# facebookresearch/ReAgent

Hardware: NVIDIA H100
Metric: minibatch_td_updates_per_sec_b4096 (higher is better)
Workload: dtype f32

## Files before the change

profiles/time_k2.py:

```python
import argparse
import json
import os
import statistics
import sys
import tempfile

ROOT = os.path.dirname(os.path.dirname(os.path.abspath(__file__)))
if ROOT not in sys.path:
    sys.path.insert(0, ROOT)

from profiles.timing import (alternate, capture, card_info, cuda_device,
                             replay_us, write_result)

CTAS = (1, 8, 32, 64, 128)
ARRANGEMENTS = {"k1_on_side_stream": True, "one_stream": False}


def k2_graph(trainer, rb, rows, A, launches):
    from reagent_b200 import _lib

    batch = rb.sample_discrete_dqn_batch(rows, A)
    trainer.train_batch(batch)
    qd, qtd, a, wsc, keep, pack = trainer._last_td_call
    assert pack is not None, "config-2 shapes run K2 on the wgmma path"
    alive = (trainer._ws, keep, batch, pack)
    lib = _lib.lib()

    def launch():
        _lib.check(lib.rb200_dqn_td_step_tc(qd, qtd, a, wsc, pack.data_ptr(), pack.numel(), 1,
                                            _lib.cur_stream()), "rb200_dqn_td_step_tc")

    return capture(launch, launches), alive


def draw(rb, n, B, dev):
    import numpy as np
    import torch

    out = np.empty((n, B), dtype=np.float64)
    for i in range(n):
        qv, pos, _ = rb.host_queries(B)
        while pos:
            qv, pos, _ = rb.host_queries(B)
        out[i] = qv
    return torch.from_numpy(out).to(dev)


def kernel_class(name):
    if "dqn_td_tc" in name:
        return "K2"
    if "wgrad" in name:
        return "wgrad"
    if "adam" in name:
        return "adam"
    if "sample" in name or "draw" in name:
        return "K1"
    return "other"


def breakdown(g, steps, tmp, tag):
    import torch
    from torch.profiler import ProfilerActivity, profile

    g.replay()
    torch.cuda.synchronize()
    with profile(activities=[ProfilerActivity.CUDA]) as prof:
        g.replay()
        torch.cuda.synchronize()
    path = os.path.join(tmp, f"k2_{tag}.pt.trace.json")
    prof.export_chrome_trace(path)
    with open(path) as f:
        ev = [e for e in json.load(f)["traceEvents"]
              if e.get("cat") == "kernel" and e.get("ph") == "X"]
    ev.sort(key=lambda e: e["ts"])
    dur, gap, last_end = {}, {}, {}
    for e in ev:
        c = kernel_class(e["name"])
        s = e.get("args", {}).get("stream", -1)
        dur.setdefault(c, []).append(e["dur"])
        if s in last_end:
            gap.setdefault(c, []).append(e["ts"] - last_end[s])
        last_end[s] = e["ts"] + e["dur"]
    k2 = [e["ts"] for e in ev if kernel_class(e["name"]) == "K2"]
    period = [b - a for a, b in zip(k2, k2[1:])]
    return {
        "kernels_per_update": {c: len(v) / steps for c, v in dur.items()},
        "names": sorted({e["name"][:120] for e in ev}),
        "median_us": {c: statistics.median(v) for c, v in dur.items()},
        "median_gap_before_on_same_stream_us": {c: statistics.median(v) for c, v in gap.items()},
        "median_k2_start_to_start_us": statistics.median(period) if period else None,
    }


def main():
    ap = argparse.ArgumentParser()
    ap.add_argument("--out", required=True, help="directory for the result file")
    ap.add_argument("--reps", type=int, default=11)
    ap.add_argument("--launches", type=int, default=200)
    ap.add_argument("--steps", type=int, default=100)
    args = ap.parse_args()

    dev = cuda_device(__file__)
    import torch

    import bench
    from reagent_b200.replay_memory import PrioritizedReplayBuffer
    from reagent_b200.training.fused_step import capture_device_only

    cfg = dict(bench.CONFIGS[2])
    B, A = cfg["B"], cfg["A"]
    info = card_info()
    rb = PrioritizedReplayBuffer(stack_size=1, replay_capacity=cfg["cap"], batch_size=B, device=dev)
    rb.add_batch(**bench.synth_stream(cfg["cap"], 1000, cfg))
    trainer = bench.build_trainer(cfg, dev)

    graphs, alive = {}, []
    for n in CTAS:
        graphs[n], keep = k2_graph(trainer, rb, 32 * n, A, args.launches)
        alive.append(keep)
    k2 = alternate(CTAS, args.reps, lambda n, rep: replay_us(graphs[n], args.launches))
    del graphs
    sweep = {str(n): {s: v[s] for s in ("median", "min", "max")} for n, v in k2.items()}

    for _ in range(3):
        trainer.train_batch(rb.sample_discrete_dqn_batch(B, A))
    torch.cuda.synchronize()
    steps = {k: capture_device_only(trainer, rb, B, args.steps, draw(rb, args.steps, B, dev),
                                    overlap_sampling=ov) for k, ov in ARRANGEMENTS.items()}
    per_update = alternate(steps, args.reps, lambda k, rep: replay_us(steps[k], args.steps))
    with tempfile.TemporaryDirectory() as tmp:
        traced = {k: breakdown(g, args.steps, tmp, k) for k, g in steps.items()}

    one, full = sweep["1"]["median"], sweep[str(CTAS[-1])]["median"]
    res = {
        "what": ("dqn_td_tc_kernel (K2) at config-2 shapes: alone at 32 rows per CTA over a "
                 "sweep of CTA counts; the captured config-2 step kernel by kernel and per "
                 "update, with the sample kernel (K1) of the next update on a second stream "
                 "(bench.py's graph) and with all kernels on one stream"),
        "card": info,
        "config": dict(B=B, S=cfg["S"], A=A, sizes=cfg["sizes"], double_q=True, loss="huber"),
        "method": (f"K2: CUDA events around one replay of a graph of {args.launches} launches "
                   f"(weights prepacked), captured after 5 warm-up launches on a side stream, "
                   f"{args.reps} alternating repetitions, medians; step: CUDA events around one "
                   f"replay of a {args.steps}-update capture_device_only graph, {args.reps} "
                   f"alternating repetitions; every timed replay after an untimed one; "
                   f"breakdown: torch.profiler (CUDA activities) over one replay of the same "
                   f"graphs, in a separate pass"),
        "k2_alone_us_by_ctas": sweep,
        "k2_128_over_1_cta": full / one,
        "step_per_update_us": per_update,
        "step_breakdown": traced,
    }
    write_result(args.out, __file__, res)


if __name__ == "__main__":
    main()
```

reagent_b200/csrc/rb200_dqn_tc.cu:

```cuda
#include <string.h>

#include "rb200_dqn_tc_layout.cuh"
#include "rb200_wgmma.cuh"

namespace rb200 {

constexpr int kQR = 32;
constexpr int kQSub = 2;
constexpr int kQStages = 3;
constexpr int kQStageBytes = kQSub * (kQKC / 4) * kQFullLbo;
constexpr int kQLboB = 64 * 16 + 16;
constexpr int kQLoOff = 32 * 4;
constexpr int kQEpiThreads = 256;
constexpr int kQThreads = kQEpiThreads + 32;
constexpr int kQMaxTiles = 4;
constexpr int kQMaxSteps = 4 * kMaxLayers;
constexpr int kQMaxSmem = 232448;
static_assert(kQKC == 32, "a chunk is four K = 8 MMA steps");

enum { kStepHidden = 0, kStepLast = 1, kStepBwd = 2 };

struct QStep {
  uint32_t pack_off;
  int16_t N, K;
  int8_t layer, kind, net, in_buf, load_x, save, qdst, out_buf;
};

struct QDev {
  rb200_dqn_args_t a;
  rb200_net_ws_t ws;
  const unsigned char* pack;
  int nsteps, last_fwd_step;
  int buf_off[3];
  int q_off, ldq, lin_off, bar_off;
  int need_zero;
  QStep steps[kQMaxSteps];
};

struct PackJob {
  const float* W;
  int N, K;
  int ld;
  int transpose;
  uint32_t pack_off;
  int chunk0;
};
struct PackDev {
  PackJob jobs[3 * kMaxLayers];
  int njobs;
  unsigned char* pack;
};

constexpr int kPackParts = 4;

__global__ void __launch_bounds__(256) dqn_tc_pack_kernel(const PackDev p) {
  const int chunk = (int)blockIdx.x / kPackParts, part = (int)blockIdx.x % kPackParts;
  int j = 0;
  while (j + 1 < p.njobs && chunk >= p.jobs[j + 1].chunk0) ++j;
  const PackJob job = p.jobs[j];
  const int local = chunk - job.chunk0;
  const int kch = ceil_div(job.K, kQKC);
  const int t = local / kch, c = local - t * kch;
  const ChunkGeo g = chunk_geo(job.N, job.K, t, c);
  const int rows8 = (int)(g.lbo - 16) / 16, kl8 = g.ksteps * 8;
  float* img = reinterpret_cast<float*>(p.pack + job.pack_off + g.off);
  const int m0 = 128 * t, k0 = kQKC * c;
  const int total = rows8 * kl8;
  constexpr int U = 4;
  for (int base = (part * 256 + (int)threadIdx.x); base < total; base += kPackParts * 256 * U) {
    float v[U];
    int o[U];
#pragma unroll
    for (int u = 0; u < U; ++u) {
      const int idx = base + u * kPackParts * 256;
      int m, kk;
      if (job.transpose) { kk = idx / rows8; m = idx - kk * rows8; }
      else { m = idx / kl8; kk = idx - m * kl8; }
      v[u] = 0.f;
      o[u] = -1;
      if (idx < total) {
        o[u] = (kk >> 2) * (int)(g.lbo / 4) + m * 4 + (kk & 3);
        if (m0 + m < job.N && k0 + kk < job.K)
          v[u] = job.transpose ? __ldg(job.W + (size_t)(k0 + kk) * job.ld + m0 + m)
                               : __ldg(job.W + (size_t)(m0 + m) * job.ld + k0 + kk);
      }
    }
#pragma unroll
    for (int u = 0; u < U; ++u)
      if (o[u] >= 0) img[o[u]] = v[u];
  }
}

__device__ __noinline__ float act_fwd_slow(float x, int act) { return act_fwd(x, act); }
__device__ __noinline__ float act_bwd_slow(float y, int act) { return act_bwd_from_out(y, act); }

template <bool kWeighted>
__global__ void __launch_bounds__(kQThreads, 1)
dqn_td_tc_kernel(const Mlp q, const Mlp qt, const QDev p) {
  extern __shared__ __align__(128) unsigned char smem_raw[];
  const int tid = threadIdx.x, warp = tid >> 5, lane = tid & 31;
  const rb200_dqn_args_t& a = p.a;
  const int B = a.batch;
  const int row0 = blockIdx.x * kQR;
  const int L = q.n_layers;
  const int A = q.dims[L];

  if (p.need_zero) {
    unsigned nbytes;
    asm("mov.u32 %0, %%dynamic_smem_size;" : "=r"(nbytes));
    for (unsigned i = (unsigned)p.buf_off[0] + tid * 16u; i + 15u < nbytes; i += kQThreads * 16u)
      *reinterpret_cast<float4*>(smem_raw + i) = make_float4(0.f, 0.f, 0.f, 0.f);
  }
  __syncthreads();

  unsigned char* ring = smem_raw;
  float* qarr = reinterpret_cast<float*>(smem_raw + p.q_off);
  float* act_s = reinterpret_cast<float*>(smem_raw + p.lin_off);
  float* mask_s = act_s + kQR * A;
  float* scal_s = mask_s + kQR * A;
  uint64_t* full = reinterpret_cast<uint64_t*>(smem_raw + p.bar_off);
  uint64_t* sfree = full + kQStages;
  const int ldq = p.ldq;

  if (tid == 0) {
    for (int s = 0; s < kQStages; ++s) { mbar_init(full + s, 1); mbar_init(sfree + s, kQEpiThreads / 32); }
    asm volatile("fence.mbarrier_init.release.cluster;\n" ::: "memory");
  }
  __syncthreads();

  const int role = __shfl_sync(0xffffffffu, warp, 0);
  if (role == kQEpiThreads / 32) {
    const bool leader = elect_one();
    int stage = 0;
    uint32_t par = 1;
    for (int s = 0; s < p.nsteps; ++s) {
      const QStep st = p.steps[s];
      const int mt = ceil_div(st.N, 128), kch = ceil_div(st.K, kQKC);
      const uint32_t tile_stride = (uint32_t)(round_up8(st.K) / 4) * kQFullLbo;
      for (int t = 0; t < mt; ++t) {
        const int rows = st.N - 128 * t;
        const uint32_t lbo = (uint32_t)(round_up8(rows < 128 ? rows : 128) * 16 + 16);
        const uint32_t full_bytes = (kQKC / 4) * lbo;
        const int klast = st.K - kQKC * (kch - 1);
        const uint32_t last_bytes = (uint32_t)(round_up8(klast) / 4) * lbo;
        const unsigned char* src = p.pack + st.pack_off + (size_t)t * tile_stride;
        for (int c = 0; c < kch; c += kQSub) {
          const int nsub = kch - c < kQSub ? kch - c : kQSub;
          const uint32_t bytes = (uint32_t)(nsub - 1) * full_bytes + ((c + nsub == kch) ? last_bytes : full_bytes);
          mbar_wait(sfree + stage, par);
          if (leader) {
            mbar_expect_tx(full + stage, bytes);
            bulk_g2s(ring + stage * kQStageBytes, src, bytes, full + stage);
          }
          src += bytes;
          if (++stage == kQStages) { stage = 0; par ^= 1u; }
        }
      }
    }
  } else {
    const int wg = warp >> 2, w4 = warp & 3, g = lane >> 2, tq = lane & 3;
    int ss = 0;
    uint32_t spar = 0;

    constexpr int kXQ = 4;
    const int xS = q.dims[0];
    const int xnq = round_up8(xS) / 4;
    const bool x_in_regs = kQR * xnq <= kXQ * kQEpiThreads;
    float4 xr[kXQ];
    auto x_fetch_one = [&](const float* src, int idx) {
      const bool vec = ((xS & 3) == 0) && ((reinterpret_cast<uintptr_t>(src) & 15) == 0);
      const int r = idx / xnq, qd = idx - r * xnq;
      const int k = 4 * qd, row = row0 + r;
      float4 v = make_float4(0.f, 0.f, 0.f, 0.f);
      if (idx < kQR * xnq && row < B) {
        const float* sp = src + (size_t)row * xS;
        if (vec && k + 3 < xS) {
          asm volatile("ld.global.nc.v4.f32 {%0,%1,%2,%3}, [%4];\n"
                       : "=f"(v.x), "=f"(v.y), "=f"(v.z), "=f"(v.w)
                       : "l"(sp + k));
        } else {
          if (k < xS) v.x = sp[k];
          if (k + 1 < xS) v.y = sp[k + 1];
          if (k + 2 < xS) v.z = sp[k + 2];
          if (k + 3 < xS) v.w = sp[k + 3];
        }
      }
      return v;
    };
    auto x_store_one = [&](int idx, const float4 v) {
      if (idx >= kQR * xnq) return;
      float* base = reinterpret_cast<float*>(smem_raw + p.buf_off[0]);
      const int r = idx / xnq, qd = idx - r * xnq;
      float4 h, l;
      split4(v, h, l);
      const int o = qd * (kQLboB / 4) + r * 4;
      *reinterpret_cast<float4*>(base + o) = h;
      *reinterpret_cast<float4*>(base + o + kQLoOff) = l;
    };
    auto x_fetch = [&](const float* src) {
      if (!x_in_regs) return;
#pragma unroll
      for (int i = 0; i < kXQ; ++i) xr[i] = x_fetch_one(src, tid + i * kQEpiThreads);
    };
    auto x_store = [&](const float* src) {
      if (x_in_regs) {
#pragma unroll
        for (int i = 0; i < kXQ; ++i) x_store_one(tid + i * kQEpiThreads, xr[i]);
      } else {
        for (int idx = tid; idx < kQR * xnq; idx += kQEpiThreads) x_store_one(idx, x_fetch_one(src, idx));
      }
    };
    auto load_loss_inputs = [&]() {
      const float* mask = a.maxq ? a.possible_next_actions_mask : a.next_action;
      for (int idx = tid; idx < kQR * A; idx += kQEpiThreads) {
        const int r = idx / A;
        const bool in = row0 + r < B;
        const size_t g = (size_t)row0 * A + idx;
        act_s[idx] = in ? a.action[g] : 0.f;
        mask_s[idx] = (in && mask) ? mask[g] : 1.f;
      }
      if (tid < kQR) {
        const int row = row0 + tid;
        const bool in = row < B;
        scal_s[tid * 4 + 0] = in ? a.reward[row] : 0.f;
        scal_s[tid * 4 + 1] = in ? a.not_terminal[row] : 0.f;
        scal_s[tid * 4 + 2] = (in && a.discount_mode == RB200_DISCOUNT_POW) ? a.discount_src[row] : 0.f;
      }
    };
    auto step_tiles = [&](const QStep& st) {
      const Mlp& net = st.net ? qt : q;
      const int l = st.layer, N = st.N;
      const int mt = ceil_div(N, 128), kch = ceil_div(st.K, kQKC);
      float* obase = reinterpret_cast<float*>(smem_raw + p.buf_off[st.out_buf]);
      const uint32_t bbase = smem_u32(smem_raw + p.buf_off[st.in_buf]);
      for (int t = 0; t < mt; ++t) {
        const int rows = N - 128 * t;
        const int rows8 = round_up8(rows < 128 ? rows : 128);
        const uint32_t lbo = (uint32_t)(rows8 * 16 + 16);
        const bool live = 64 * wg < rows;
        const int m0 = 64 * wg + 16 * w4 + g;
        const bool ok0 = live && m0 < rows8, ok1 = live && m0 + 8 < rows8;
        float acc[32];
#pragma unroll
        for (int i = 0; i < 32; ++i) acc[i] = 0.f;
        for (int c = 0; c < kch; c += kQSub) {
          const int nsub = kch - c < kQSub ? kch - c : kQSub;
          mbar_wait(full + ss, spar);
          uint32_t ah[kQSub * 4][4], al[kQSub * 4][4];
          int ksteps[kQSub];
#pragma unroll
          for (int j = 0; j < kQSub; ++j) {
            const int kl = st.K - kQKC * (c + j);
            ksteps[j] = j < nsub ? round_up8(kl < kQKC ? kl : kQKC) / 8 : 0;
            const unsigned char* src = ring + ss * kQStageBytes + (uint32_t)j * (kQKC / 4) * lbo + tq * 4;
#pragma unroll
            for (int ks = 0; ks < 4; ++ks) {
              float v[4] = {0.f, 0.f, 0.f, 0.f};
              if (ks < ksteps[j]) {
                const unsigned char* s0 = src + (uint32_t)(2 * ks) * lbo;
                const unsigned char* s1 = s0 + lbo;
                if (ok0) { v[0] = *reinterpret_cast<const float*>(s0 + m0 * 16); v[2] = *reinterpret_cast<const float*>(s1 + m0 * 16); }
                if (ok1) { v[1] = *reinterpret_cast<const float*>(s0 + (m0 + 8) * 16); v[3] = *reinterpret_cast<const float*>(s1 + (m0 + 8) * 16); }
              }
#pragma unroll
              for (int e = 0; e < 4; ++e) {
                float h, lo_;
                split1(v[e], h, lo_);
                ah[4 * j + ks][e] = __float_as_uint(h);
                al[4 * j + ks][e] = __float_as_uint(lo_);
              }
            }
          }
          __syncwarp();
          if (lane == 0) mbar_arrive(sfree + ss);
          if (++ss == kQStages) { ss = 0; spar ^= 1u; }
          wgmma_fence();
#pragma unroll
          for (int j = 0; j < kQSub; ++j) {
#pragma unroll
            for (int ks = 0; ks < 4; ++ks) {
              if (ks < ksteps[j]) {
                const uint32_t kq = (uint32_t)(2 * (4 * (c + j) + ks));
                const uint64_t bd = wgmma_desc(bbase + kq * kQLboB, kQLboB, 128);
                wgmma_rs_n64(acc, ah[4 * j + ks], bd, 1u);
                wgmma_rs_n32(acc, al[4 * j + ks], bd, 1u);
              }
            }
          }
          wgmma_commit();
          wgmma_wait<0>();
        }
        if (!live) continue;

#pragma unroll
        for (int hh = 0; hh < 2; ++hh) {
          const int n = 128 * t + m0 + 8 * hh;
          const bool valid = n < N;
          float x[8];
#pragma unroll
          for (int i = 0; i < 4; ++i)
#pragma unroll
            for (int e = 0; e < 2; ++e) x[2 * i + e] = acc[4 * i + 2 * hh + e] + acc[4 * (i + 4) + 2 * hh + e];
          auto rowof = [&](int k) { return 8 * (k >> 1) + 2 * tq + (k & 1); };
          float* ob = obase + (n >> 2) * (kQLboB / 4) + (n & 3);
          bool to_operand, to_global;
          float* gdst = nullptr;
          if (st.kind == kStepBwd) {
            const int hact = q.act[l - 1];
            float hv[8];
            if (st.save) {
              const float* hs = p.ws.hidden[l - 1];
#pragma unroll
              for (int k = 0; k < 8; ++k) {
                const int row = row0 + rowof(k);
                hv[k] = (valid && row < B) ? hs[(size_t)row * N + n] : 0.f;
              }
            } else {
#pragma unroll
              for (int k = 0; k < 8; ++k) hv[k] = valid ? ob[rowof(k) * 4] + ob[rowof(k) * 4 + kQLoOff] : 0.f;
            }
            if (hact == RB200_ACT_RELU) {
#pragma unroll
              for (int k = 0; k < 8; ++k) x[k] = hv[k] > 0.f ? x[k] : 0.f;
            } else if (hact != RB200_ACT_LINEAR) {
#pragma unroll
              for (int k = 0; k < 8; ++k) x[k] = valid ? x[k] * act_bwd_slow(hv[k], hact) : 0.f;
            }
            to_operand = l - 1 >= 1;
            to_global = true;
            gdst = p.ws.dz[l - 1];
          } else {
            const float bias = valid ? __ldg(net.params + net.b_off[l] + n) : 0.f;
            const int act = net.act[l];
            if (act == RB200_ACT_RELU) {
#pragma unroll
              for (int k = 0; k < 8; ++k) x[k] = fmaxf(x[k] + bias, 0.f);
            } else if (act == RB200_ACT_LINEAR) {
#pragma unroll
              for (int k = 0; k < 8; ++k) x[k] += bias;
            } else {
#pragma unroll
              for (int k = 0; k < 8; ++k) x[k] = act_fwd_slow(x[k] + bias, act);
            }
            to_operand = st.kind != kStepLast;
            to_global = st.save != 0 && st.kind != kStepLast;
            gdst = to_global ? p.ws.hidden[l] : nullptr;
          }
          if (!valid) continue;
          if (st.kind == kStepLast) {
            float* qd = qarr + st.qdst * kQR * ldq + n;
#pragma unroll
            for (int k = 0; k < 8; ++k) qd[rowof(k) * ldq] = x[k];
            continue;
          }
          if (to_operand) {
#pragma unroll
            for (int k = 0; k < 8; ++k) {
              float h, lo_;
              split1(row0 + rowof(k) < B ? x[k] : 0.f, h, lo_);
              ob[rowof(k) * 4] = h;
              ob[rowof(k) * 4 + kQLoOff] = lo_;
            }
          }
          if (to_global) {
#pragma unroll
            for (int k = 0; k < 8; ++k) {
              const int row = row0 + rowof(k);
              if (row < B) gdst[(size_t)row * N + n] = x[k];
            }
          }
        }
      }
    };
    auto loss_stage = [&]() {
      const float* qa = qarr;
      const float* qb = qarr + kQR * ldq;
      const float* qc = qarr + 2 * kQR * ldq;
      const int r = tid >> 3, sub = tid & 7;
      const int row = row0 + r;
      const bool in = row < B;
      float best = 0.f, sel = 0.f, qsel = 0.f, bsum = 0.f;
      int bi = 0x7fffffff;
      for (int c = sub; c < A; c += 8) {
        const float pen = -1e9f * (1.f - mask_s[r * A + c]);
        const float vt = qb[r * ldq + c] + pen;
        const float key = a.double_q ? (qa[r * ldq + c] + pen) : vt;
        if (bi == 0x7fffffff || key > best) { best = key; bi = c; sel = vt; }
        const float aw = act_s[r * A + c];
        qsel += qc[r * ldq + c] * aw;
        if (a.reward_boost) bsum += aw * a.reward_boost[c];
      }
#pragma unroll
      for (int o = 1; o < 8; o <<= 1) {
        const float ob = __shfl_xor_sync(0xffffffffu, best, o);
        const float os = __shfl_xor_sync(0xffffffffu, sel, o);
        const int oi = __shfl_xor_sync(0xffffffffu, bi, o);
        qsel += __shfl_xor_sync(0xffffffffu, qsel, o);
        bsum += __shfl_xor_sync(0xffffffffu, bsum, o);
        if (oi != 0x7fffffff && (bi == 0x7fffffff || ob > best || (ob == best && oi < bi))) {
          best = ob; bi = oi; sel = os;
        }
      }
      float le = 0.f, g = 0.f;
      if (in) {
        const float rew = scal_s[r * 4 + 0] + bsum;
        const float disc = (a.discount_mode == RB200_DISCOUNT_POW)
                               ? powf(a.gamma, scal_s[r * 4 + 2]) : a.gamma;
        const float tgt = rew + disc * (sel * scal_s[r * 4 + 1]);
        const float d = qsel - tgt;
        const float invB = 1.f / (float)B;
        if (a.loss_kind == RB200_LOSS_HUBER) {
          const float ad = fabsf(d);
          le = ad < 1.f ? 0.5f * d * d : ad - 0.5f;
          g = (d < -1.f) ? -invB : (d > 1.f ? invB : invB * d);
        } else {
          le = d * d;
          g = 2.f * invB * d;
        }
        if (kWeighted) {
          const float w = a.sample_weight[row];
          le *= w;
          g *= w;
        }
        if (sub == 0) {
          if (a.td_target) a.td_target[row] = tgt;
          if (a.next_action_idx) a.next_action_idx[row] = bi;
          if (a.q_selected) a.q_selected[row] = qsel;
        }
      }
      const int A8 = round_up8(A);
      const int lact = q.act[L - 1];
      float* zb = reinterpret_cast<float*>(smem_raw + p.buf_off[2]) + r * 4;
      for (int c = sub; c < A8; c += 8) {
        float v = 0.f;
        if (in && c < A) {
          v = g * act_s[r * A + c];
          if (lact != RB200_ACT_LINEAR) v *= act_bwd_slow(qc[r * ldq + c], lact);
          if (a.all_action_scores) a.all_action_scores[(size_t)row * A + c] = qc[r * ldq + c];
          if (a.do_backward) p.ws.dz[L - 1][(size_t)row * A + c] = v;
        }
        if (a.do_backward) {
          float h, lo_;
          split1(v, h, lo_);
          float* o = zb + (c >> 2) * (kQLboB / 4) + (c & 3);
          o[0] = h;
          o[kQLoOff] = lo_;
        }
      }
      const float ws = warp_sum(sub == 0 ? le : 0.f);
      if (lane == 0) scal_s[kQR * 4 + warp] = ws;
    };


    auto x_src = [&](int lx) { return lx == 1 ? a.state : a.next_state; };
    auto handover = [&]() {
      fence_proxy_async_smem();
      asm volatile("bar.sync 1, %0;\n" ::"n"(kQEpiThreads) : "memory");
    };
    if (p.steps[0].load_x) { x_fetch(x_src(p.steps[0].load_x)); x_store(x_src(p.steps[0].load_x)); }
    load_loss_inputs();
    handover();
    for (int s = 0; s < p.nsteps; ++s) {
      const QStep st = p.steps[s];
      const int lx = (s + 1 < p.nsteps) ? p.steps[s + 1].load_x : 0;
      if (lx) x_fetch(x_src(lx));
      step_tiles(st);
      handover();
      if (s == p.last_fwd_step) {
        loss_stage();
        handover();
      }
      if (lx) {
        x_store(x_src(lx));
        handover();
      }
    }

    if (tid == 0) {
      float loss_partial = 0.f;
      for (int w = 0; w < kQEpiThreads / 32; ++w) loss_partial += scal_s[kQR * 4 + w];
      finish_serial<1>(a.loss_partials, a.tile_counter, {loss_partial},
                       [&](const float (&tot)[1]) { *a.loss = tot[0] / (float)B; });
    }
  }
}

struct QPlan {
  QDev dev;
  PackDev pack;
  int pack_chunks;
  size_t smem_bytes;
  int64_t pack_bytes;
  bool ok;
};

static QPlan make_plan(const rb200_mlp_t* qn, const rb200_mlp_t* qtn, int double_q, int do_backward) {
  QPlan pl;
  memset(&pl, 0, sizeof(pl));
  pl.ok = false;
  const int L = qn->n_layers;
  if (L < 1 || L > kMaxLayers) return pl;
  for (int l = 1; l <= L; ++l)
    if (qn->dims[l] > 128 * kQMaxTiles || qn->dims[l] > 32000) return pl;
  if (qn->dims[0] > 32000 || qn->dims[L] > 256) return pl;

  uint32_t off = 0;
  uint32_t off_on[kMaxLayers], off_tg[kMaxLayers], off_bw[kMaxLayers];
  int nj = 0, nchunks = 0;
  auto add_job = [&](const rb200_mlp_t* net, int l, int transpose) {
    PackJob& j = pl.pack.jobs[nj++];
    j.W = net->params + net->w_off[l];
    j.ld = net->dims[l];
    j.transpose = transpose;
    j.N = transpose ? net->dims[l] : net->dims[l + 1];
    j.K = transpose ? net->dims[l + 1] : net->dims[l];
    j.pack_off = off;
    j.chunk0 = nchunks;
    nchunks += ceil_div(j.N, 128) * ceil_div(j.K, kQKC);
    const uint32_t o = off;
    off += image_bytes(j.N, j.K);
    return o;
  };
  for (int l = 0; l < L; ++l) off_on[l] = add_job(qn, l, 0);
  if (qtn) for (int l = 0; l < L; ++l) off_tg[l] = add_job(qtn, l, 0);
  else for (int l = 0; l < L; ++l) { off_tg[l] = off; off += image_bytes(qn->dims[l + 1], qn->dims[l]); nj++; }
  if (do_backward) for (int l = 1; l < L; ++l) off_bw[l] = add_job(qn, l, 1);
  pl.pack.njobs = nj;
  pl.pack_chunks = nchunks;
  {
    const TcImages im = tc_images(qn, do_backward);
    pl.pack_bytes = im.total_bytes;
    bool same = im.total_bytes == (int64_t)off + 4096;
    for (int l = 0; l < L; ++l) same = same && im.on_fwd[l] == off_on[l] && im.tg_fwd[l] == off_tg[l];
    if (do_backward) for (int l = 1; l < L; ++l) same = same && im.on_bwd[l] == off_bw[l];
    if (!same) return pl;
  }

  int ns = 0;
  auto add_pass = [&](int net, int load_x, int save, int qdst) {
    for (int l = 0; l < L; ++l) {
      QStep& s = pl.dev.steps[ns++];
      s.pack_off = net ? off_tg[l] : off_on[l];
      s.N = (int16_t)qn->dims[l + 1];
      s.K = (int16_t)qn->dims[l];
      s.layer = (int8_t)l;
      s.kind = (l == L - 1) ? kStepLast : kStepHidden;
      s.net = (int8_t)net;
      s.in_buf = (int8_t)(l & 1);
      s.out_buf = (int8_t)((l + 1) & 1);
      s.load_x = (int8_t)(l == 0 ? load_x : 0);
      s.save = (int8_t)save;
      s.qdst = (int8_t)qdst;
    }
  };
  add_pass(1, 2, 0, 1);
  if (double_q) add_pass(0, 2, 0, 0);
  add_pass(0, 1, do_backward ? 1 : 0, 2);
  pl.dev.last_fwd_step = ns - 1;
  if (do_backward) {
    for (int l = L - 1; l >= 1; --l) {
      QStep& s = pl.dev.steps[ns++];
      s.pack_off = off_bw[l];
      s.N = (int16_t)qn->dims[l];
      s.K = (int16_t)qn->dims[l + 1];
      s.layer = (int8_t)l;
      s.kind = kStepBwd;
      s.net = 0;
      s.in_buf = (int8_t)(l == L - 1 ? 2 : ((l + 1) & 1));
      s.out_buf = (int8_t)(l & 1);
      s.save = (int8_t)(l <= L - 3 ? 1 : 0);
    }
  }
  pl.dev.nsteps = ns;
  pl.dev.need_zero = 0;
  for (int l = 0; l <= L; ++l)
    if (qn->dims[l] % 8 != 0) pl.dev.need_zero = 1;

  int maxd[3] = {8, 8, qn->dims[L]};
  for (int i = 0; i < L; ++i) if (qn->dims[i] > maxd[i & 1]) maxd[i & 1] = qn->dims[i];
  size_t o = (size_t)kQStages * kQStageBytes;
  for (int b = 0; b < 3; ++b) {
    pl.dev.buf_off[b] = (int)o;
    o += (size_t)(round_up8(maxd[b]) / 4) * kQLboB;
  }
  pl.dev.ldq = qn->dims[L] + 1;
  pl.dev.q_off = (int)o;
  o += (size_t)3 * kQR * pl.dev.ldq * sizeof(float);
  o = (o + 15) & ~(size_t)15;
  pl.dev.lin_off = (int)o;
  o += ((size_t)2 * kQR * qn->dims[L] + 4 * kQR + 8) * sizeof(float);
  o = (o + 15) & ~(size_t)15;
  pl.dev.bar_off = (int)o;
  o += 2 * kQStages * sizeof(uint64_t);
  pl.smem_bytes = (o + 15) & ~(size_t)15;
  pl.ok = pl.smem_bytes <= (size_t)kQMaxSmem;
  return pl;
}

}

using namespace rb200;

extern "C" int64_t rb200_dqn_tc_workspace_bytes(const rb200_mlp_t* q_net, int32_t double_q,
                                                int32_t do_backward) {
  if (!q_net || validate_mlp(q_net, "q_network")) return 0;
  const QPlan pl = make_plan(q_net, nullptr, double_q, do_backward);
  return pl.ok ? pl.pack_bytes : 0;
}

extern "C" int rb200_dqn_tc_pack(const rb200_mlp_t* q_net, const rb200_mlp_t* q_target,
                                 int32_t double_q, int32_t do_backward, void* pack_ws,
                                 int64_t pack_ws_bytes, void* stream) {
  if (!q_net || !q_target || !pack_ws) { set_last_error("rb200_dqn_tc_pack: null argument"); return RB200_E_INVALID; }
  if (int rc = validate_mlp(q_net, "q_network")) return rc;
  if (int rc = validate_mlp(q_target, "q_network_target")) return rc;
  if (q_net->n_layers != q_target->n_layers) { set_last_error("q_network / target layer count mismatch"); return RB200_E_INVALID; }
  for (int l = 0; l <= q_net->n_layers; ++l)
    if (q_net->dims[l] != q_target->dims[l]) { set_last_error("q_network / target dims mismatch at %d", l); return RB200_E_INVALID; }
  if ((reinterpret_cast<uintptr_t>(pack_ws) & 127) != 0) { set_last_error("pack workspace must be 128-byte aligned"); return RB200_E_INVALID; }
  QPlan pl = make_plan(q_net, q_target, double_q, do_backward);
  if (!pl.ok) { set_last_error("rb200_dqn_tc_pack: shapes do not fit the wgmma path"); return RB200_E_SMEM; }
  if (pack_ws_bytes < pl.pack_bytes) { set_last_error("pack workspace too small: %lld < %lld", (long long)pack_ws_bytes, (long long)pl.pack_bytes); return RB200_E_INVALID; }
  pl.pack.pack = static_cast<unsigned char*>(pack_ws);
  dqn_tc_pack_kernel<<<pl.pack_chunks * kPackParts, 256, 0, (cudaStream_t)stream>>>(pl.pack);
  return check_cuda(cudaGetLastError(), "dqn_tc_pack_kernel launch");
}

extern "C" int rb200_dqn_td_step_tc(const rb200_mlp_t* q_net, const rb200_mlp_t* q_target,
                                    const rb200_dqn_args_t* args, const rb200_net_ws_t* ws,
                                    void* pack_ws, int64_t pack_ws_bytes, int32_t weights_packed,
                                    void* stream) {
  if (!q_net || !q_target || !args || !ws || !pack_ws) { set_last_error("rb200_dqn_td_step_tc: null argument"); return RB200_E_INVALID; }
  if (!weights_packed) {
    if (int rc = rb200_dqn_tc_pack(q_net, q_target, args->double_q, args->do_backward, pack_ws, pack_ws_bytes, stream)) return rc;
  }
  if (int rc = validate_mlp(q_net, "q_network")) return rc;
  if (int rc = validate_mlp(q_target, "q_network_target")) return rc;
  if (q_net->n_layers != q_target->n_layers) { set_last_error("q_network / target layer count mismatch"); return RB200_E_INVALID; }
  for (int l = 0; l <= q_net->n_layers; ++l)
    if (q_net->dims[l] != q_target->dims[l]) { set_last_error("q_network / target dims mismatch at %d", l); return RB200_E_INVALID; }
  if (args->batch <= 0) { set_last_error("batch must be positive"); return RB200_E_INVALID; }
  if (!args->state || !args->next_state || !args->action || !args->reward || !args->not_terminal ||
      !args->loss_partials || !args->loss || !args->tile_counter) {
    set_last_error("rb200_dqn_td_step_tc: required pointer is null"); return RB200_E_INVALID;
  }
  if (!args->maxq && !args->next_action) { set_last_error("SARSA update needs next_action"); return RB200_E_INVALID; }
  if (args->discount_mode == RB200_DISCOUNT_POW && !args->discount_src) { set_last_error("POW discount needs discount_src"); return RB200_E_INVALID; }
  if (args->do_backward) {
    for (int l = 0; l < q_net->n_layers; ++l)
      if (!ws->dz[l] || (l < q_net->n_layers - 1 && !ws->hidden[l])) { set_last_error("workspace buffer missing for layer %d", l); return RB200_E_INVALID; }
  }
  if ((reinterpret_cast<uintptr_t>(pack_ws) & 127) != 0) { set_last_error("pack workspace must be 128-byte aligned"); return RB200_E_INVALID; }
  QPlan pl = make_plan(q_net, q_target, args->double_q, args->do_backward);
  if (!pl.ok) { set_last_error("rb200_dqn_td_step_tc: shapes do not fit the wgmma path"); return RB200_E_SMEM; }
  if (pack_ws_bytes < pl.pack_bytes) { set_last_error("pack workspace too small: %lld < %lld", (long long)pack_ws_bytes, (long long)pl.pack_bytes); return RB200_E_INVALID; }
  pl.dev.a = *args;
  pl.dev.ws = *ws;
  pl.dev.pack = static_cast<const unsigned char*>(pack_ws);
  cudaStream_t st = (cudaStream_t)stream;
  const bool weighted = args->sample_weight != nullptr;
  if (cudaError_t e = weighted ? opt_in_smem<dqn_td_tc_kernel<true>>(pl.smem_bytes)
                               : opt_in_smem<dqn_td_tc_kernel<false>>(pl.smem_bytes))
    return check_cuda(e, "cudaFuncSetAttribute(dqn_td_tc)");
  static int greatest[64] = {};
  static bool have_greatest[64] = {};
  int dev = 0;
  if (cudaError_t e = cudaGetDevice(&dev)) return check_cuda(e, "cudaGetDevice");
  int prio = 0;
  if (dev >= 0 && dev < 64 && have_greatest[dev]) {
    prio = greatest[dev];
  } else {
    int least = 0;
    if (cudaError_t e = cudaDeviceGetStreamPriorityRange(&least, &prio))
      return check_cuda(e, "cudaDeviceGetStreamPriorityRange");
    if (dev >= 0 && dev < 64) { greatest[dev] = prio; have_greatest[dev] = true; }
  }
  const Mlp q = make_mlp(q_net), qt = make_mlp(q_target);
  cudaLaunchConfig_t cfg = {};
  cfg.gridDim = dim3((unsigned)ceil_div(args->batch, kQR));
  cfg.blockDim = dim3(kQThreads);
  cfg.dynamicSmemBytes = pl.smem_bytes;
  cfg.stream = st;
  cudaLaunchAttribute attr[1];
  attr[0].id = cudaLaunchAttributePriority;
  attr[0].val.priority = prio;
  cfg.attrs = attr;
  cfg.numAttrs = 1;
  const cudaError_t e = weighted ? cudaLaunchKernelEx(&cfg, dqn_td_tc_kernel<true>, q, qt, pl.dev)
                                 : cudaLaunchKernelEx(&cfg, dqn_td_tc_kernel<false>, q, qt, pl.dev);
  return check_cuda(e, "dqn_td_tc_kernel launch");
}
```

reagent_b200/csrc/rb200_wgmma.cuh:

```cuda
#pragma once
#include "rb200_common.cuh"

namespace rb200 {

__device__ __forceinline__ uint32_t smem_u32(const void* p) {
  return static_cast<uint32_t>(__cvta_generic_to_shared(p));
}

__device__ __forceinline__ uint64_t wgmma_desc(uint32_t saddr, uint32_t lbo_bytes, uint32_t sbo_bytes) {
  uint64_t d = 0;
  d |= (uint64_t)((saddr >> 4) & 0x3fff);
  d |= (uint64_t)((lbo_bytes >> 4) & 0x3fff) << 16;
  d |= (uint64_t)((sbo_bytes >> 4) & 0x3fff) << 32;
  return d;
}

__device__ __forceinline__ void wgmma_fence() { asm volatile("wgmma.fence.sync.aligned;\n" ::: "memory"); }
__device__ __forceinline__ void wgmma_commit() { asm volatile("wgmma.commit_group.sync.aligned;\n" ::: "memory"); }
template <int N>
__device__ __forceinline__ void wgmma_wait() {
  asm volatile("wgmma.wait_group.sync.aligned %0;\n" ::"n"(N) : "memory");
}

__device__ __forceinline__ void mbar_init(uint64_t* bar, uint32_t count) {
  asm volatile("mbarrier.init.shared::cta.b64 [%0], %1;\n" ::"r"(smem_u32(bar)), "r"(count));
}
__device__ __forceinline__ void mbar_wait(uint64_t* bar, uint32_t parity) {
  const uint32_t addr = smem_u32(bar);
  for (long long it = 0;; ++it) {
    uint32_t ok;
    asm volatile(
        "{\n\t"
        ".reg .pred p;\n\t"
        "mbarrier.try_wait.parity.shared::cta.b64 p, [%1], %2;\n\t"
        "selp.u32 %0, 1, 0, p;\n\t"
        "}\n"
        : "=r"(ok)
        : "r"(addr), "r"(parity)
        : "memory");
    if (ok) break;
    if (it > 400000LL) __trap();
  }
}

__device__ __forceinline__ void split4(const float4 v, float4& hi, float4& lo) {
  uint32_t h;
  h = (__float_as_uint(v.x) + 0x1000u) & 0xffffe000u; hi.x = __uint_as_float(h); lo.x = v.x - hi.x;
  h = (__float_as_uint(v.y) + 0x1000u) & 0xffffe000u; hi.y = __uint_as_float(h); lo.y = v.y - hi.y;
  h = (__float_as_uint(v.z) + 0x1000u) & 0xffffe000u; hi.z = __uint_as_float(h); lo.z = v.z - hi.z;
  h = (__float_as_uint(v.w) + 0x1000u) & 0xffffe000u; hi.w = __uint_as_float(h); lo.w = v.w - hi.w;
}
__device__ __forceinline__ void split1(float x, float& hi, float& lo) {
  hi = __uint_as_float((__float_as_uint(x) + 0x1000u) & 0xffffe000u);
  lo = x - hi;
}

__device__ __forceinline__ void mbar_arrive(uint64_t* bar) {
  asm volatile("mbarrier.arrive.shared::cta.b64 _, [%0];\n" ::"r"(smem_u32(bar)) : "memory");
}
__device__ __forceinline__ void mbar_expect_tx(uint64_t* bar, uint32_t bytes) {
  asm volatile("mbarrier.arrive.expect_tx.shared::cta.b64 _, [%0], %1;\n" ::"r"(smem_u32(bar)),
               "r"(bytes)
               : "memory");
}
__device__ __forceinline__ void bulk_g2s(void* smem_dst, const void* gsrc, uint32_t bytes,
                                         uint64_t* bar) {
  asm volatile(
      "cp.async.bulk.shared::cluster.global.mbarrier::complete_tx::bytes [%0], [%1], %2, [%3];\n" ::
          "r"(smem_u32(smem_dst)),
      "l"(gsrc), "r"(bytes), "r"(smem_u32(bar))
      : "memory");
}
__device__ __forceinline__ void fence_proxy_async_smem() {
  asm volatile("fence.proxy.async.shared::cta;\n" ::: "memory");
}
__device__ __forceinline__ bool elect_one() {
  uint32_t pred;
  asm volatile(
      "{\n\t"
      ".reg .pred p;\n\t"
      "elect.sync _|p, 0xffffffff;\n\t"
      "selp.u32 %0, 1, 0, p;\n\t"
      "}\n"
      : "=r"(pred));
  return pred != 0;
}

__device__ __forceinline__ void wgmma_ss_n128(float* d, uint64_t da, uint64_t db, uint32_t accumulate) {
  asm volatile(
      "{\n\t.reg .pred p;\n\tsetp.ne.b32 p, %66, 0;\n\t"
      "wgmma.mma_async.sync.aligned.m64n128k8.f32.tf32.tf32 {%0,%1,%2,%3,%4,%5,%6,%7,%8,%9,%10,%11,%12,%13,%14,%15,%16,%17,%18,%19,%20,%21,%22,%23,%24,%25,%26,%27,%28,%29,%30,%31,%32,%33,%34,%35,%36,%37,%38,%39,%40,%41,%42,%43,%44,%45,%46,%47,%48,%49,%50,%51,%52,%53,%54,%55,%56,%57,%58,%59,%60,%61,%62,%63}, %64, %65, p, 1, 1;\n\t}\n"
      : "+f"(d[0]), "+f"(d[1]), "+f"(d[2]), "+f"(d[3]), "+f"(d[4]), "+f"(d[5]), "+f"(d[6]), "+f"(d[7]), "+f"(d[8]), "+f"(d[9]), "+f"(d[10]), "+f"(d[11]), "+f"(d[12]), "+f"(d[13]), "+f"(d[14]), "+f"(d[15]), "+f"(d[16]), "+f"(d[17]), "+f"(d[18]), "+f"(d[19]), "+f"(d[20]), "+f"(d[21]), "+f"(d[22]), "+f"(d[23]), "+f"(d[24]), "+f"(d[25]), "+f"(d[26]), "+f"(d[27]), "+f"(d[28]), "+f"(d[29]), "+f"(d[30]), "+f"(d[31]), "+f"(d[32]), "+f"(d[33]), "+f"(d[34]), "+f"(d[35]), "+f"(d[36]), "+f"(d[37]), "+f"(d[38]), "+f"(d[39]), "+f"(d[40]), "+f"(d[41]), "+f"(d[42]), "+f"(d[43]), "+f"(d[44]), "+f"(d[45]), "+f"(d[46]), "+f"(d[47]), "+f"(d[48]), "+f"(d[49]), "+f"(d[50]), "+f"(d[51]), "+f"(d[52]), "+f"(d[53]), "+f"(d[54]), "+f"(d[55]), "+f"(d[56]), "+f"(d[57]), "+f"(d[58]), "+f"(d[59]), "+f"(d[60]), "+f"(d[61]), "+f"(d[62]), "+f"(d[63])
      : "l"(da), "l"(db), "r"(accumulate));
}

__device__ __forceinline__ void wgmma_rs_n32(float* d, const uint32_t (&a)[4], uint64_t db, uint32_t accumulate) {
  asm volatile(
      "{\n\t.reg .pred p;\n\tsetp.ne.b32 p, %21, 0;\n\t"
      "wgmma.mma_async.sync.aligned.m64n32k8.f32.tf32.tf32 {%0,%1,%2,%3,%4,%5,%6,%7,%8,%9,%10,%11,%12,%13,%14,%15}, {%16,%17,%18,%19}, %20, p, 1, 1;\n\t}\n"
      : "+f"(d[0]), "+f"(d[1]), "+f"(d[2]), "+f"(d[3]), "+f"(d[4]), "+f"(d[5]), "+f"(d[6]), "+f"(d[7]), "+f"(d[8]), "+f"(d[9]), "+f"(d[10]), "+f"(d[11]), "+f"(d[12]), "+f"(d[13]), "+f"(d[14]), "+f"(d[15])
      : "r"(a[0]), "r"(a[1]), "r"(a[2]), "r"(a[3]), "l"(db), "r"(accumulate));
}

__device__ __forceinline__ void wgmma_rs_n64(float* d, const uint32_t (&a)[4], uint64_t db, uint32_t accumulate) {
  asm volatile(
      "{\n\t.reg .pred p;\n\tsetp.ne.b32 p, %37, 0;\n\t"
      "wgmma.mma_async.sync.aligned.m64n64k8.f32.tf32.tf32 {%0,%1,%2,%3,%4,%5,%6,%7,%8,%9,%10,%11,%12,%13,%14,%15,%16,%17,%18,%19,%20,%21,%22,%23,%24,%25,%26,%27,%28,%29,%30,%31}, {%32,%33,%34,%35}, %36, p, 1, 1;\n\t}\n"
      : "+f"(d[0]), "+f"(d[1]), "+f"(d[2]), "+f"(d[3]), "+f"(d[4]), "+f"(d[5]), "+f"(d[6]), "+f"(d[7]), "+f"(d[8]), "+f"(d[9]), "+f"(d[10]), "+f"(d[11]), "+f"(d[12]), "+f"(d[13]), "+f"(d[14]), "+f"(d[15]), "+f"(d[16]), "+f"(d[17]), "+f"(d[18]), "+f"(d[19]), "+f"(d[20]), "+f"(d[21]), "+f"(d[22]), "+f"(d[23]), "+f"(d[24]), "+f"(d[25]), "+f"(d[26]), "+f"(d[27]), "+f"(d[28]), "+f"(d[29]), "+f"(d[30]), "+f"(d[31])
      : "r"(a[0]), "r"(a[1]), "r"(a[2]), "r"(a[3]), "l"(db), "r"(accumulate));
}

}
```

Measured before the change: 9916.

## Double-buffer wgmma A fragments to overlap smem fetch with in-flight MMAs

```diff
diff --git a/profiles/time_k2.py b/profiles/time_k2.py
--- a/profiles/time_k2.py
+++ b/profiles/time_k2.py
@@ -2,6 +2,7 @@
 import json
 import os
 import statistics
+import subprocess
 import sys
 import tempfile
 
@@ -92,13 +93,58 @@
     }
 
 
+def headline(res):
+    k2 = res["k2_alone_us_by_ctas"]
+    return {"k2_alone_us_1_cta": k2["1"]["median"], f"k2_alone_us_{CTAS[-1]}_ctas": k2[str(CTAS[-1])]["median"],
+            **{f"step_us_{k}": v["median"] for k, v in res["step_per_update_us"].items()},
+            "k2_us_in_step_k1_on_side_stream": res["step_breakdown"]["k1_on_side_stream"]["median_us"]["K2"]}
+
+
+def against(args):
+    libs = {"this_tree": None, "against": args.against}
+    runs = {k: [] for k in libs}
+    with tempfile.TemporaryDirectory() as tmp:
+        for r in range(args.runs):
+            for k in (list(libs) if r % 2 == 0 else list(libs)[::-1]):
+                env = dict(os.environ)
+                env.pop("RB200_LIB", None)
+                if libs[k]:
+                    env["RB200_LIB"] = os.path.abspath(libs[k])
+                out = os.path.join(tmp, f"{k}_{r}")
+                subprocess.run([sys.executable, os.path.abspath(__file__), "--out", out, "--reps", str(args.reps),
+                                "--launches", str(args.launches), "--steps", str(args.steps)],
+                               env=env, check=True, stdout=subprocess.DEVNULL)
+                (name,) = os.listdir(out)
+                with open(os.path.join(out, name)) as f:
+                    runs[k].append(json.load(f))
+    first = runs["this_tree"][0]
+    res = {
+        "what": first["what"] + f"; {args.runs} runs with each of two libraries, alternating",
+        "card": first["card"],
+        "cards_of_all_runs": sorted({json.dumps(x["card"]) for v in runs.values() for x in v}),
+        "libraries": {k: v or "the tree's reagent_b200/libreagent_b200.so" for k, v in libs.items()},
+        "config": first["config"],
+        "method": first["method"] + "; each run a separate process, the two libraries alternating",
+        "median_over_runs": {k: {h: statistics.median(headline(x)[h] for x in v) for h in headline(v[0])}
+                             for k, v in runs.items()},
+        "min_max_over_runs": {k: {h: [min(headline(x)[h] for x in v), max(headline(x)[h] for x in v)]
+                                  for h in headline(v[0])} for k, v in runs.items()},
+        "runs": {k: [headline(x) for x in v] for k, v in runs.items()},
+    }
+    write_result(args.out, "time_k2_against", res)
+
+
 def main():
     ap = argparse.ArgumentParser()
     ap.add_argument("--out", required=True, help="directory for the result file")
     ap.add_argument("--reps", type=int, default=11)
     ap.add_argument("--launches", type=int, default=200)
     ap.add_argument("--steps", type=int, default=100)
+    ap.add_argument("--against", metavar="LIB", help="another build of libreagent_b200.so to compare with")
+    ap.add_argument("--runs", type=int, default=5, help="runs per library with --against")
     args = ap.parse_args()
+    if args.against:
+        return against(args)
 
     dev = cuda_device(__file__)
     import torch
diff --git a/reagent_b200/csrc/rb200_dqn_tc.cu b/reagent_b200/csrc/rb200_dqn_tc.cu
--- a/reagent_b200/csrc/rb200_dqn_tc.cu
+++ b/reagent_b200/csrc/rb200_dqn_tc.cu
@@ -1,4 +1,6 @@
 #include <string.h>
+
+#include <type_traits>
 
 #include "rb200_dqn_tc_layout.cuh"
 #include "rb200_wgmma.cuh"
@@ -93,6 +95,26 @@
 
 __device__ __noinline__ float act_fwd_slow(float x, int act) { return act_fwd(x, act); }
 __device__ __noinline__ float act_bwd_slow(float y, int act) { return act_bwd_from_out(y, act); }
+
+constexpr int kQCK = kQKC / 8;
+
+template <int NK>
+__device__ __forceinline__ void chunk_mma(float (&acc)[32], const uint32_t (&ah)[kQCK][4],
+                                          const uint32_t (&al)[kQCK][4], uint32_t b0) {
+  wgmma_fence();
+#pragma unroll
+  for (int kk = 0; kk < NK; ++kk) {
+    const uint64_t bd = wgmma_desc(b0 + (uint32_t)(2 * kk) * kQLboB, kQLboB, 128);
+    wgmma_rs_n64(acc, ah[kk], bd, 1u);
+    wgmma_rs_n32(acc, al[kk], bd, 1u);
+  }
+  wgmma_commit();
+}
+template <int NK, typename F>
+__device__ __forceinline__ void with_ksteps(int nk, F&& f) {
+  if (nk == NK) f(std::integral_constant<int, NK>());
+  else if constexpr (NK > 1) with_ksteps<NK - 1>(nk, f);
+}
 
 template <bool kWeighted>
 __global__ void __launch_bounds__(kQThreads, 1)
@@ -242,54 +264,64 @@
         const bool ok0 = live && m0 < rows8, ok1 = live && m0 + 8 < rows8;
         float acc[32];
 #pragma unroll
-        for (int i = 0; i < 32; ++i) acc[i] = 0.f;
-        for (int c = 0; c < kch; c += kQSub) {
-          const int nsub = kch - c < kQSub ? kch - c : kQSub;
-          mbar_wait(full + ss, spar);
-          uint32_t ah[kQSub * 4][4], al[kQSub * 4][4];
-          int ksteps[kQSub];
-#pragma unroll
-          for (int j = 0; j < kQSub; ++j) {
-            const int kl = st.K - kQKC * (c + j);
-            ksteps[j] = j < nsub ? round_up8(kl < kQKC ? kl : kQKC) / 8 : 0;
-            const unsigned char* src = ring + ss * kQStageBytes + (uint32_t)j * (kQKC / 4) * lbo + tq * 4;
-#pragma unroll
-            for (int ks = 0; ks < 4; ++ks) {
-              float v[4] = {0.f, 0.f, 0.f, 0.f};
-              if (ks < ksteps[j]) {
-                const unsigned char* s0 = src + (uint32_t)(2 * ks) * lbo;
-                const unsigned char* s1 = s0 + lbo;
-                if (ok0) { v[0] = *reinterpret_cast<const float*>(s0 + m0 * 16); v[2] = *reinterpret_cast<const float*>(s1 + m0 * 16); }
-                if (ok1) { v[1] = *reinterpret_cast<const float*>(s0 + (m0 + 8) * 16); v[3] = *reinterpret_cast<const float*>(s1 + (m0 + 8) * 16); }
-              }
-#pragma unroll
-              for (int e = 0; e < 4; ++e) {
-                float h, lo_;
-                split1(v[e], h, lo_);
-                ah[4 * j + ks][e] = __float_as_uint(h);
-                al[4 * j + ks][e] = __float_as_uint(lo_);
-              }
+        for (int i = 0; i < 32; ++i) {
+          acc[i] = 0.f;
+          wgmma_fence_operand(acc[i]);
+        }
+        static_assert(kQSub == 2, "one fragment buffer per chunk of a ring stage");
+        const int kfull = st.K / kQKC;
+        const int nk_last = round_up8(st.K - kQKC * kfull) / 8;
+        uint32_t ah[2][kQCK][4], al[2][kQCK][4];
+        auto fetch = [&](uint32_t (&fh)[kQCK][4], uint32_t (&fl)[kQCK][4], int c, int nk) {
+          if (c % 2 == 0) mbar_wait(full + ss, spar);
+          float v[kQCK][4];
+#pragma unroll
+          for (int kk = 0; kk < kQCK; ++kk) {
+            v[kk][0] = v[kk][1] = v[kk][2] = v[kk][3] = 0.f;
+            const unsigned char* s0 = ring + ss * kQStageBytes + (uint32_t)((c % 2) * (kQKC / 4) + 2 * kk) * lbo + tq * 4;
+            const unsigned char* s1 = s0 + lbo;
+            if (kk < nk && ok0) { v[kk][0] = *reinterpret_cast<const float*>(s0 + m0 * 16); v[kk][2] = *reinterpret_cast<const float*>(s1 + m0 * 16); }
+            if (kk < nk && ok1) { v[kk][1] = *reinterpret_cast<const float*>(s0 + (m0 + 8) * 16); v[kk][3] = *reinterpret_cast<const float*>(s1 + (m0 + 8) * 16); }
+          }
+          if (c % 2 == 1 || c + 1 == kch) {
+            __syncwarp();
+            if (lane == 0) mbar_arrive(sfree + ss);
+            if (++ss == kQStages) { ss = 0; spar ^= 1u; }
+          }
+#pragma unroll
+          for (int kk = 0; kk < kQCK; ++kk)
+#pragma unroll
+            for (int e = 0; e < 4; ++e) {
+              float h, lo_;
+              split1(v[kk][e], h, lo_);
+              fh[kk][e] = __float_as_uint(h);
+              fl[kk][e] = __float_as_uint(lo_);
+              wgmma_fence_operand(fh[kk][e]);
+              wgmma_fence_operand(fl[kk][e]);
             }
-          }
-          __syncwarp();
-          if (lane == 0) mbar_arrive(sfree + ss);
-          if (++ss == kQStages) { ss = 0; spar ^= 1u; }
-          wgmma_fence();
-#pragma unroll
-          for (int j = 0; j < kQSub; ++j) {
-#pragma unroll
-            for (int ks = 0; ks < 4; ++ks) {
-              if (ks < ksteps[j]) {
-                const uint32_t kq = (uint32_t)(2 * (4 * (c + j) + ks));
-                const uint64_t bd = wgmma_desc(bbase + kq * kQLboB, kQLboB, 128);
-                wgmma_rs_n64(acc, ah[4 * j + ks], bd, 1u);
-                wgmma_rs_n32(acc, al[4 * j + ks], bd, 1u);
-              }
-            }
-          }
-          wgmma_commit();
+        };
+        auto b_of = [&](int c) { return bbase + (uint32_t)(2 * kQCK * c) * kQLboB; };
+        if (kfull > 0) fetch(ah[0], al[0], 0, kQCK);
+        for (int c = 0; c < kfull; c += 2) {
+          chunk_mma<kQCK>(acc, ah[0], al[0], b_of(c));
+          if (c + 1 == kfull) break;
+          wgmma_wait<1>();
+          fetch(ah[1], al[1], c + 1, kQCK);
+          chunk_mma<kQCK>(acc, ah[1], al[1], b_of(c + 1));
+          if (c + 2 == kfull) break;
+          wgmma_wait<1>();
+          fetch(ah[0], al[0], c + 2, kQCK);
+        }
+        if (kfull < kch) {
           wgmma_wait<0>();
-        }
+          fetch(ah[0], al[0], kfull, nk_last);
+          with_ksteps<kQCK>(nk_last, [&](auto nk_c) {
+            chunk_mma<decltype(nk_c)::value>(acc, ah[0], al[0], b_of(kfull));
+          });
+        }
+        wgmma_wait<0>();
+#pragma unroll
+        for (int i = 0; i < 32; ++i) wgmma_fence_operand(acc[i]);
         if (!live) continue;
 
 #pragma unroll
diff --git a/reagent_b200/csrc/rb200_wgmma.cuh b/reagent_b200/csrc/rb200_wgmma.cuh
--- a/reagent_b200/csrc/rb200_wgmma.cuh
+++ b/reagent_b200/csrc/rb200_wgmma.cuh
@@ -21,6 +21,8 @@
 __device__ __forceinline__ void wgmma_wait() {
   asm volatile("wgmma.wait_group.sync.aligned %0;\n" ::"n"(N) : "memory");
 }
+__device__ __forceinline__ void wgmma_fence_operand(uint32_t& r) { asm volatile("" : "+r"(r)::"memory"); }
+__device__ __forceinline__ void wgmma_fence_operand(float& r) { asm volatile("" : "+f"(r)::"memory"); }
 
 __device__ __forceinline__ void mbar_init(uint64_t* bar, uint32_t count) {
   asm volatile("mbarrier.init.shared::cta.b64 [%0], %1;\n" ::"r"(smem_u32(bar)), "r"(count));
```

Result: faster. 10670, median of 6 (+7.6%).
